# JuliaMolSim/Molly.jl

Measured on AMD Instinct MI355X. Metric: ns_per_day, higher is better.
Workload: dtype f32; 1 GPU; 1M-atom LJ fluid (argon, rho=21.1/nm3), cubic PBC, DistanceCutoff 1.0 nm, r_list 1.2 nm, dt 2 fs, VelocityVerlet, remove_CM_motion=1; integrator=vv, n_atoms=1000000, rebuild_every=10, parallelism=single domain, block_atoms=256, j_split=2, pairs_half_list=75841147

## Files before the change

### molly.jl_amd/csrc/engine.hip

```cpp
#include <algorithm>
#include <chrono>
#include <cstddef>
#include <cstdlib>
#include <cstring>
#include <limits>
#include <memory>
#include <new>
#include <string>
#include <vector>

#include <unistd.h>

#include "bonded.h"
#include "stochastic.h"
#include "constraints.h"
#include "virtual_sites.h"
#include "pme.h"
#include "step_fused.h"
#include "hilbert.h"
#include "kernels.h"
#include "list_policy.h"
#include "replan.h"
#include "halo_step.h"
#include "forces_launch.h"
// ... 715 lines not shown
        case MHIP_COUL_PLAIN: go(std::integral_constant<int, MHIP_COUL_PLAIN>{}); break;
        case MHIP_COUL_REACTION_FIELD: go(std::integral_constant<int, MHIP_COUL_REACTION_FIELD>{}); break;
        default: if (I.approx_erfc) go(std::integral_constant<int, MHIP_COUL_EWALD_DIRECT>{}); else go(std::integral_constant<int, COUL_EWALD_EXACT>{}); break;
        }
    }
    struct PassReq {
        bool step = false;
        bool gcv = false;
        bool cm = false, measure = false;
        double dt = 0;
        const StochP<T>* lang = nullptr;
        bool halo = false, halo_cm_in = false;
        bool fuse_spread = false, fuse_terms = false;
        const double* cm_sum_in = nullptr;
        T4* frc = nullptr;
    };
    struct PassRes {
        bool step = false; int parts = 0;
        bool gs = false, spread = false, terms = false;
        bool cm_summed = false;
    };
    PassShape pass_shape(bool energy, int part, bool allow_gs, const PassReq& req) {
        PassShape s;
        s.fp32 = std::is_same<T, float>::value; s.ljm = ljm; s.coulm = coulm; s.minimg = minimg; s.n_special = n_special > 0 ? 1 : 0; s.eshift = eshift; s.lj_c12 = I.lj_c12 != T(0);
        s.BI = BI; s.JS = JS; s.T_cap = T_cap; s.lds_budget = (size_t)env_int("MOLLYHIP_LDS_BUDGET_KB", 160) * 1024;
        s.dual = dual; s.inner_valid = inner_valid; s.max_tile = max_tile; s.max_tile_in = max_tile_in;
        s.gs = gs_groups(); s.gs_list_current = gs_list_id == n_filters; s.n_ghost = n_ghost;
        s.energy = energy; s.part = part; s.allow_gs = allow_gs; s.own_frc = req.frc != nullptr;
        s.step = req.step; s.halo = req.halo; s.fuse_step = fuse_step_env;
        s.cm_mode = pending_cm.mode(); s.cm_n = pending_cm.n; s.in_step_loop = in_vv_fused || in_lang_fused;
        return s;
    }
    static void throw_capacity(const PassPlan& plan) { if (plan.capacity != PassCapacity::OK) throw ApiError{MHIP_ERR_CAPACITY, capacity_message(plan.capacity)}; }

    PassRes launch_pair_kernel(bool energy, int part = 0, bool allow_gs = false, const PassReq& req = PassReq{}) {
        prune_resolve(!(xf_direct && n_ghost > 0));
        if constexpr (std::is_same<T, float>::value) {
            if (dual && !inner_valid && !energy && allow_gs && part == 0 && !req.frc && adopt_env && gs_groups() > 0 && cnt_outer_valid && margin_zero && !(lp.skin_in < lp.skin)
                && lp.last_outer_step == pass_step && n_ghost == 0 && !host_prune) adopt_outer_list();
        }
        const PassPlan plan = plan_pass(pass_shape(energy, part, allow_gs, req));
        throw_capacity(plan);
        if (req.halo && !plan.steps) throw ApiError{MHIP_ERR_STATE, "internal: the fused ghosted step was asked for a pass that cannot integrate"};
        if (plan.form == PassForm::GROUP_SPLIT) return launch_gs_pass(plan, req);
        last_plan = plan;
        PassRes res;
        ForceArgs<T> A{};
        fill_block_args(A, plan, part, req.frc);
        if (plan.prune) arm_prune(A, plan);
        if (plan.cm_fin) { cm_fin_buf.reserve(4); A.cm_fin_in = pending_cm.parts_arg(); A.cm_fin_n = pending_cm.n; A.cm_fin_out = cm_fin_buf.p; }
        else if (req.cm_sum_in && plan.cm_slot) {
            cm_fin_buf.reserve(4); A.cm_fin_in = req.cm_sum_in; A.cm_fin_n = pending_cm.n; A.cm_fin_out = cm_fin_buf.p; res.cm_summed = true;
        }
        A.dbg = (!plan.prune && !energy) ? stamps_begin((size_t)n_blocks * 16 * 8) : nullptr;
        if (plan.steps) arm_step(A, req);
        prof.begin(plan.prune ? 4 : 0, stream);
        tr(plan.prune ? "k_forces (prune)" : (energy ? "k_forces (energy)" : (plan.steps ? (req.halo ? "k_forces (fused ghosted step)" : "k_forces (fused step)") : "k_forces")));
        launch_block_pass(A, plan, energy, req);
        if (plan.steps) { res.step = true; res.parts = n_blocks; }
        if (plan.cm_fin) pending_cm.moved(cm_fin_buf.p, 1);
        tr("after k_forces");
        if (plan.prune && gs_groups() > 0) {
            regroup(nbr_in.p, cnt_in.p, tile_cnt_in.p, false);
            gs_list_id = n_filters + 1;
        }
        prof.end(plan.prune ? 4 : 0, stream);
        MHIP_HIP(hipGetLastError());
        ++n_force_calls;
        if (A.dbg && (n_force_calls % stamps_every()) == 0) stamps_report();
        if (plan.prune) finish_prune(xf_direct && n_ghost > 0 && prune_late_env);
        return res;
    }

    PassRes launch_gs_pass(const PassPlan& plan, const PassReq& req) {
        PassRes res;
        if constexpr (std::is_same<T, float>::value) {
            const int GS = gs_groups();
            frc_parts.reserve((size_t)(GS - 1) * cap);
            GsArgs Z{};
            Z.G = G; Z.I = I; Z.n_owned = n_owned; Z.BI = BI; Z.BI_shift = ilog2(BI); Z.JS = JS; Z.GS = GS; Z.lgGS = ilog2(GS); Z.R_cap = GS * R_cap;
            Z.T_cap = T_cap; Z.Q_lds = plan.q_lds; Z.n_blocks = n_blocks; Z.spread = std::max(1, n_blocks / GS + 5);
            Z.pos = pos[cur].p; Z.lj = lj[cur].p; Z.tile_idx = inner_is_outer ? tile_idx.p : tile_idx_in.p; Z.tile_cnt = inner_is_outer ? tile_cnt.p : tile_cnt_in.p; Z.nbr = nbr_gs.p; Z.wave_rows = rows_gs.p; Z.blk_center = blk_center.p;
            Z.frc = frc[cur].p; Z.parts = frc_parts.p; Z.part_stride = cap; Z.item_of = gs_item.p;
            Z.dbg = stamps_begin((size_t)n_blocks * GS * 4 * 8);
            last_plan.tile_max = plan.tile_max;
            prof.begin(0, stream);
            tr("k_forces_gs");
            if (req.fuse_spread || req.fuse_terms) {
                bonded.ensure_roles(stream, cap);
                const int order = req.fuse_spread ? pme.order : 5;
                if (plan.cm_fin) cm_fin_buf.reserve(4);
                const size_t lds = (req.fuse_spread ? std::max(plan.lds_bytes, std::min<size_t>((size_t)MAX_LDS_BYTES / GS, spread_head_bytes_f32(order) + (size_t)PME_BOX_BYTES)) : plan.lds_bytes) & ~(size_t)15;
                const int n_spread = req.fuse_spread ? (int)std::min<int64_t>(cdiv(n_owned, (int64_t)64), 4096) : 0;
                launch_pair_spread_bonded(Z, n_blocks * GS, coulm, minimg, order, n_owned, reinterpret_cast<float*>(pme.rgrid.p), reinterpret_cast<const PmeP<float>&>(pme.P), n_spread,
                                          reinterpret_cast<const BondedArgs<float>&>(static_cast<const BondedArgs<T>&>(bonded.slot_args(G, I, pos[cur].p, inv.p))), cdiv(bonded.n_blocks(), 4), lds, stream,
                                          plan.cm_fin ? pending_cm.parts_arg() : (const double*)nullptr, pending_cm.n, plan.cm_fin ? cm_fin_buf.p : (double*)nullptr);
                if (plan.cm_fin) pending_cm.moved(cm_fin_buf.p, 1);
                res.spread = req.fuse_spread; res.terms = !req.fuse_spread;
            } else launch_forces_gs(Z, coulm, minimg, stream);
            prof.end(0, stream);
            MHIP_HIP(hipGetLastError());
            ++n_force_calls; ++n_gs_passes; res.gs = true;
            if (Z.dbg && (n_gs_passes % stamps_every()) == 0) stamps_dump("", (size_t)n_blocks * GS * 4 * 8);
        }
        return res;
    }

    void fill_block_args(ForceArgs<T>& A, const PassPlan& plan, int part, T4* own_frc) {
        A.G = G; A.I = I; A.n_owned = n_owned; A.BI = BI; A.BI_shift = ilog2(BI); A.JS = JS; A.T_cap = T_cap; A.T_lds = plan.tile_lds; A.R_cap = R_cap;
        A.n_blocks = n_blocks; A.blocks_per_xcd = cdiv(n_blocks, 8);
        A.pos = pos[cur].p; A.lj = lj[cur].p; A.blk_center = blk_center.p; A.frc = own_frc ? own_frc : frc[cur].p; A.pe_part = red_part.p;
        const bool pruned = plan.use_inner && !inner_is_outer;
        A.tile_idx = pruned ? tile_idx_in.p : tile_idx.p; A.tile_cnt = pruned ? tile_cnt_in.p : tile_cnt.p;
        A.nbr = pruned ? nbr_in.p : nbr.p; A.wave_rows = pruned ? wave_rows_in.p : wave_rows.p;
        A.r_prune2 = r_prune2; A.any_special = n_special > 0 ? 1 : 0; A.eshift = eshift; A.soa = plan.soa;
        if (part != 0 && !plan.prune) {
            DBuf<int32_t>& fl = plan.use_inner ? blk_ghost_in : blk_ghost; bool& ok = plan.use_inner ? ghost_flags_in_ok : ghost_flags_ok;
            if (!ok) {
                fl.reserve(n_blocks);
                hipLaunchKernelGGL(k_block_ghost_flags, dim3(n_blocks), dim3(WAVE), 0, stream, n_blocks, T_cap, n_owned, (const int32_t*)A.tile_idx, (const int32_t*)A.tile_cnt, fl.p);
                ok = true;
            }
// ... 197 lines not shown
        gs_item.reserve((size_t)n_blocks * GS);
        launch_gs_balance((const int32_t*)rows_gs.p, n_blocks, JS, GS, BI / WAVE, cu_count, gs_item.p, stream);
    }

    void adopt_outer_list() {
        prof.begin(4, stream);
        pos_snap_in.reserve(cap);
        MHIP_HIP(hipMemcpyAsync(pos_snap_in.p, pos[cur].p, (size_t)n_tot * sizeof(T4), hipMemcpyDeviceToDevice, stream));
        regroup(nbr.p, cnt_outer.p, tile_cnt.p, true);
        prof.end(4, stream);
        MHIP_HIP(hipGetLastError());
        inner_is_outer = true; max_tile_in = max_tile; lp.last_prune_step = pass_step;
        ++n_filters; ++n_adopted; gs_list_id = n_filters;
        ghost_flags_in_ok = false; lp.next_check_step = -1; hx.tile_ok = false;
        inner_valid = true; prune_disp_exceeded = false;
        if (debug_on) std::fprintf(stderr, "[mhip] outer list adopted as the inner list (no prune): rows %lld calls %lld\n", (long long)total_rows, (long long)n_force_calls);
    }

#if MHIP_STAMPS
    DBuf<unsigned long long> dbg_buf;
    static int stamps_every() { static const int n = env_int("MOLLYHIP_DBG_TIMES", 0); return std::max(n, 1); }
    unsigned long long* stamps_begin(size_t words) {
        static const int on = env_int("MOLLYHIP_DBG_TIMES", 0);
        if (!on) return nullptr;
        dbg_buf.reserve(words); MHIP_HIP(hipMemsetAsync(dbg_buf.p, 0, words * sizeof(unsigned long long), stream));
        return dbg_buf.p;
    }
    void stamps_dump(const char* suffix, size_t words) {
        std::vector<unsigned long long> h(words);
        MHIP_HIP(hipStreamSynchronize(stream));
        MHIP_HIP(hipMemcpy(h.data(), dbg_buf.p, h.size() * sizeof(unsigned long long), hipMemcpyDeviceToHost));
        if (const char* path = std::getenv("MOLLYHIP_DBG_DUMP")) { if (FILE* f = std::fopen((std::string(path) + suffix).c_str(), "wb")) { std::fwrite(h.data(), sizeof(unsigned long long), h.size(), f); std::fclose(f); } }
    }
    void stamps_report() {
        const int nw = BI * JS / WAVE;
        std::vector<unsigned long long> h((size_t)n_blocks * nw * 8);
        MHIP_HIP(hipStreamSynchronize(stream));
        MHIP_HIP(hipMemcpy(h.data(), dbg_buf.p, h.size() * sizeof(unsigned long long), hipMemcpyDeviceToHost));
        unsigned long long w0 = ~0ull, w3 = 0; double sum[3] = {0, 0, 0}, mx[3] = {0, 0, 0}, clk = 0; int n = 0;
        std::vector<double> loop_us;
        for (size_t q = 0; q < (size_t)n_blocks * nw; ++q) {
            const unsigned long long* d = &h[q * 8];
            if (!d[7]) continue;
            w0 = std::min(w0, d[4]); w3 = std::max(w3, d[7]);
            for (int k = 0; k < 3; ++k) { const double us = (double)(d[5 + k] - d[4 + k]) * 0.01; sum[k] += us; mx[k] = std::max(mx[k], us); }
            loop_us.push_back((double)(d[6] - d[5]) * 0.01);
            if (d[7] > d[4]) clk += (double)(d[3] - d[0]) / ((double)(d[7] - d[4]) * 10.0);
            ++n;
        }
        std::sort(loop_us.begin(), loop_us.end());
        std::fprintf(stderr, "[mhip dbg] pair kernel: %d waves, first entry -> last exit %.2f us | per wave mean (max) us: staging %.2f (%.2f) row walk %.2f (%.2f) reduce+store %.2f (%.2f) | row walk p10 %.2f p50 %.2f p90 %.2f | shader clock %.3f GHz\n",
                     n, (double)(w3 - w0) * 0.01, sum[0] / n, mx[0], sum[1] / n, mx[1], sum[2] / n, mx[2], loop_us[n / 10], loop_us[n / 2], loop_us[(size_t)n * 9 / 10], clk / n);
    }
#else
    static int stamps_every() { return 1; }
    unsigned long long* stamps_begin(size_t) { return nullptr; }
    void stamps_dump(const char*, size_t) {}
    void stamps_report() {}
#endif
    double read_sum(int n_part) {
        hipLaunchKernelGGL(k_sum_double, dim3(1), dim3(256), 0, stream, n_part, (const double*)red_part.p, red_out.p);
        MHIP_HIP(hipMemcpyAsync(h_red, red_out.p, sizeof(double), hipMemcpyDeviceToHost, stream));
        MHIP_HIP(hipStreamSynchronize(stream));
        return h_red[0];
    }

    void export_frc(int accumulate, void* f_xyz, int mem_kind) {
        const size_t cnt = 3 * (size_t)n_owned;
        if (mem_kind == MHIP_MEM_DEVICE) {
            hipLaunchKernelGGL(k_export_forces<T>, dim3(cdiv(n_owned, 256)), dim3(256), 0, stream, n_owned, (const int32_t*)orig[cur].p, (const T4*)frc[cur].p, (T*)f_xyz, accumulate);
        } else {
            stage_a.reserve(cnt);
            if (accumulate) MHIP_HIP(hipMemcpyAsync(stage_a.p, f_xyz, cnt * sizeof(T), hipMemcpyHostToDevice, stream));
            hipLaunchKernelGGL(k_export_forces<T>, dim3(cdiv(n_owned, 256)), dim3(256), 0, stream, n_owned, (const int32_t*)orig[cur].p, (const T4*)frc[cur].p, stage_a.p, accumulate);
            MHIP_HIP(hipMemcpyAsync(f_xyz, stage_a.p, cnt * sizeof(T), hipMemcpyDeviceToHost, stream));
            MHIP_HIP(hipStreamSynchronize(stream));
        }
        MHIP_HIP(hipGetLastError());
    }

    PassRes step_forces(int64_t step_n, PassReq req = PassReq{}) {
        pass_step = step_n;
        if (pme.on() && n_ghost > 0) throw ApiError{MHIP_ERR_UNSUPPORTED, "PME runs on a single domain (SURVEY §8(e): 6mrr-size systems are replicas only)"};
        const bool gs_ok = bonded.any() && n_ghost == 0;
        const bool small_fused = bonded.any() && pme.on() && n_ghost == 0;
        req.fuse_spread = gs_ok && small_fused && pme.order >= 4 && pme.order <= 6 && !prof.on;
        req.fuse_terms = gs_ok && !small_fused && !pme.on() && !prof.on;
        PassRes res = launch_pair_kernel(false, interior_done ? 2 : 0, gs_ok, req);
        interior_done = false;
        bool redo = false;
        if (prune_disp_exceeded) {
            after_forces(step_n);
            req.fuse_spread = req.fuse_terms = false;
            if (res.cm_summed) req.cm_sum_in = nullptr;
            const PassRes again = launch_pair_kernel(false, 0, false, req);
            res.step = again.step; res.parts = again.parts; res.gs = again.gs; res.cm_summed |= again.cm_summed;
            redo = true;
        }
        if (res.gs) bonded.fold(frc_parts.p, gs_groups() - 1, cap);
        pend_a = nullptr;
        if (small_fused) {
            frc_side.reserve(cap);
            GcvArgs<T> V; const GcvArgs<T>* vp = nullptr;
            if (req.gcv && fuse_gcv_env && !redo && (pending_cm.mode() == 0 || (pending_cm.mode() == 2 && pending_cm.n == 1)) && pme.order >= 4 && pme.order <= 6) {
                const int nb = (int)Pme<T>::atom_blocks(n_owned);
                cm_blk.reserve(2 * 4 * (size_t)nb + 8);
                if (req.measure) trk_reserve(nb);
                std::memset(&V, 0, sizeof(V));
                V.vel = vel[cur].p; V.dt = T(req.dt); V.dt2 = T(req.dt) / T(2); V.G = G;
                V.cm_in = pending_cm.parts_arg();
                V.cm_out = req.cm ? cm_blk.p + (size_t)step_half * 4 * nb : (double*)nullptr;
// ... 1681 lines not shown
```

### molly.jl_amd/csrc/kernels.h

```cpp
#pragma once
#include <type_traits>
#include "pass_plan.h"
#include "physics.h"
#include "halo_xfer.h"
#include "philox.h"
#include "thermostat_step.h"

namespace mhip {

enum { FLAG_MINIMG = 0, FLAG_OVERFLOW = 1, FLAG_MAX_TILE = 2, FLAG_MAX_ROWS = 3, FLAG_NAN = 4, FLAG_TOTAL_ROWS = 5, FLAG_MAX_CELLS = 6, FLAG_MAX_DISP2 = 7, FLAG_MAX_V2 = 8, N_FLAGS = 10 };
enum { OVF_TILE = 1, OVF_ROWS = 2, OVF_BOXCELLS = 4, OVF_SLOT = 8 };

constexpr int MAX_BOX_CELLS = 8192;
constexpr uint32_t XL_EXCLUDED = 1u << 30, XL_SPECIAL = 1u << 31, XL_INDEX = (1u << 30) - 1u;

constexpr int SLOT_MAX_SCALED = 16383;
__host__ __device__ inline uint32_t entry_slot(uint32_t e, int sh) { return sh ? (e >> sh) : (e & 0x7fffu); }
__host__ __device__ inline uint32_t entry_special(uint32_t e, int sh) { return sh ? 0u : (e >> 15); }
__host__ __device__ inline uint32_t make_entry(uint32_t slot, uint32_t sp, int sh) { return sh ? (slot << sh) : (slot | (sp << 15)); }

template <class T> __device__ inline int cell_coord(T x, int d, const GridP<T>& G) {
    T rel = G.periodic[d] ? x : x - G.origin[d];
    int c = (int)M<T>::floor(rel * G.inv_cs[d]);
    return min(max(c, 0), G.nc[d] - 1);
// ... 1102 lines not shown
    double a[4] = {0, 0, 0, 0};
    for (int q = threadIdx.x; q < n_part; q += blockDim.x) { const double* p = part + 4 * (int64_t)q; a[0] += p[0]; a[1] += p[1]; a[2] += p[2]; a[3] += p[3]; }
#pragma unroll
    for (int o = 32; o > 0; o >>= 1) for (int c = 0; c < 4; ++c) a[c] += __shfl_xor(a[c], o, 64);
    double* sh = reinterpret_cast<double*>(smem);
    if ((threadIdx.x & 63) == 0) for (int c = 0; c < 4; ++c) sh[4 * (threadIdx.x >> 6) + c] = a[c];
    __syncthreads();
    if (threadIdx.x < 4) { double t = 0; for (int q = 0; q < (int)(blockDim.x >> 6); ++q) t += sh[4 * q + threadIdx.x]; out4[threadIdx.x] = t; }
    __syncthreads();
}

#ifndef MHIP_FAST_MIN_WAVES
#define MHIP_FAST_MIN_WAVES 8
#endif
#ifndef MHIP_SB
#define MHIP_SB 4
#endif
template <class T, int LJM, int COULM, bool ENERGY, bool MINIMG, bool SEG, bool PRUNE>
constexpr int force_min_waves() { return (std::is_same<T, float>::value && LJM == LJ_DIST_UNIFORM && COULM == MHIP_COUL_NONE && !ENERGY && !MINIMG && !SEG && !PRUNE) ? MHIP_FAST_MIN_WAVES : 1; }

template <class T, int LJM, int COULM, bool ENERGY, bool MINIMG, bool SEG, bool PRUNE, int SOA_STRIDE = 4097, bool STEP = false, bool HALO = false, bool LANG = false>
__global__ void __launch_bounds__(BlockLimits<T>::max_threads, (force_min_waves<T, LJM, COULM, ENERGY, MINIMG, SEG, PRUNE>()))
k_forces(ForceArgs<T> A) {
    static_assert(!HALO || (STEP && std::is_same<T, float>::value), "the ghosted form exists for the fused fp32 step only");
    static_assert(!LANG || (STEP && !HALO), "the Langevin update rides in the fused single-domain step only");
    using T4 = typename Vec<T>::T4;
    using T2 = typename Vec<T>::T2;
    constexpr bool PER_ATOM_LJ = (LJM == LJ_DIST || LJM == LJ_GENERIC);
    extern __shared__ __align__(32) unsigned char smem[];
    const GridP<T>& G = A.G;
    int wg = blockIdx.x;
    if constexpr (STEP) {
        if (wg == 0) {
            if constexpr (HALO) { if (A.cm_in) halo_cm_publish(A.H, A.cm_pub, A.step_seq, smem); }
            else if (A.cm_in) step_cm_publish(A.cm_in, A.cm_n, A.cm_pub, A.step_seq, smem);
            return;
        }
        --wg;
    }
    int b = (wg & 7) * A.blocks_per_xcd + (wg >> 3);
    [[maybe_unused]] int hflags = 0;
    if constexpr (HALO) { b = A.H.order[wg]; if (b < 0) return; hflags = A.H.flags[b]; }
    else {
        if (b >= A.n_blocks) return;
        if (A.part != 0 && (A.blk_ghost[b] != 0) != (A.part == 2)) return;
    }
    const int tid = threadIdx.x, nthr = blockDim.x;
    [[maybe_unused]] auto stamp = [&](int k) {
        if constexpr (MHIP_STAMPS != 0 && !PRUNE) {
            if (A.dbg && (tid & 63) == 0) { unsigned long long* d = A.dbg + ((size_t)b * (nthr >> 6) + (tid >> 6)) * 8; d[k] = __builtin_readcyclecounter(); d[4 + k] = wall_clock64(); }
        }
    };
    stamp(0);
    const int tile_n = A.tile_cnt[b];
    T4* l_pos = reinterpret_cast<T4*>(smem);
    T2* l_lj = reinterpret_cast<T2*>(l_pos + (A.T_lds + 1));
    const T4 ctr = A.blk_center[b];
    constexpr bool MAY_SCALE = std::is_same<T, float>::value && LJM == LJ_DIST_UNIFORM && COULM == MHIP_COUL_NONE;
    const int esh = MAY_SCALE ? A.eshift : 0;

    auto localise = [&](T4 p, auto tri_tag) -> T4 {
        if constexpr (!MINIMG) local_xyz_t<decltype(tri_tag)::value>(p.x, p.y, p.z, ctr, G);
        return p;
    };
    constexpr bool NO_TRI = std::is_same<T, float>::value && LJM == LJ_DIST_UNIFORM && COULM == MHIP_COUL_NONE && !ENERGY;
    const bool tri_local = !MINIMG && !NO_TRI && G.tri_grid;
    const int li = tid & (A.BI - 1), js = tid >> A.BI_shift;
    const int64_t si = (int64_t)b * A.BI + li;
    const bool valid = si < A.n_owned;
    [[maybe_unused]] auto step_lane = [&]() -> int { int t = tid; asm volatile("" : "+v"(t)); return t & (A.BI - 1); };
    [[maybe_unused]] auto step_atom = [&]() -> int64_t { return (int64_t)b * A.BI + step_lane(); };
    T4 pi_raw;
    if constexpr (PRUNE || COULM != MHIP_COUL_NONE) pi_raw = A.pos[valid ? si : (int64_t)b * A.BI];
    else {
        const T* own = reinterpret_cast<const T*>(A.pos + (valid ? si : (int64_t)b * A.BI));
        pi_raw = make4<T>(own[0], own[1], own[2], T(0));
    }
    T4 pi;
    T2 lji_raw = make2<T>(T(0), T(0)), lji = lji_raw;
    if constexpr (PER_ATOM_LJ) lji_raw = A.lj[valid ? si : (int64_t)b * A.BI];
    constexpr bool PRE_E = PER_ATOM_LJ && sizeof(T) == 4;
    auto pre_e = [](T2 v) { if constexpr (PRE_E) { v.y = v.x == T(0) ? T(0) : M<T>::sqrt(v.y); v.x *= T(0.5); } return v; };
    const int rows_lane = A.wave_rows[(b * A.JS + js) * (A.BI >> 6) + (li >> 6)];
    int rows = 0;
    bool own_done = false;
    auto own_ready = [&]() {
        if (own_done) return;
        own_done = true;
        if constexpr (NO_TRI) pi = localise(pi_raw, std::false_type{});
        else pi = tri_local ? localise(pi_raw, std::true_type{}) : localise(pi_raw, std::false_type{});
        lji = pre_e(lji_raw);
        rows = __builtin_amdgcn_readfirstlane(rows_lane);
    };
    if constexpr (PRUNE) own_ready();
    const uint2* my_rows = A.nbr + (((int64_t)b * A.JS + js) * A.R_cap) * A.BI + li;
    const int32_t* tix = (HALO ? A.H.tsrc : A.tile_idx) + (int64_t)b * A.T_cap;
    if constexpr (HALO) { if (hflags & 1) halo_wait_block(A.H); }
    T fx = T(0), fy = T(0), fz = T(0), pe = T(0);
    [[maybe_unused]] T vir[6] = {T(0), T(0), T(0), T(0), T(0), T(0)};
    uint64_t acc = 0;
    int kept = 0;
    uint2* out_rows = nullptr;
    if constexpr (PRUNE) out_rows = A.nbr_dst + (((int64_t)b * A.JS + js) * A.R_cap) * A.BI + li;
    [[maybe_unused]] uint16_t* l_new = nullptr; [[maybe_unused]] int32_t* l_scan = nullptr; [[maybe_unused]] float* l_box = nullptr;
    [[maybe_unused]] int32_t* l_cnt = nullptr; [[maybe_unused]] int32_t* l_wmax = nullptr; [[maybe_unused]] const uint2* l_lut = nullptr;
    [[maybe_unused]] int n_new = 0;
// ... 65 lines not shown
                        if constexpr (HALO) {
                            if (s[k] >= 0) p[k] = A.pos[s[k]];
                            else { const float* gr = A.H.rows + 3 * (size_t)(-1 - s[k]); p[k] = make4<T>((T)peer_row_load(gr), (T)peer_row_load(gr + 1), (T)peer_row_load(gr + 2), T(0)); }
                        } else p[k] = A.pos[s[k]];
                    }
#pragma unroll
                    for (int k = 0; k < SB; ++k) {
                        const int t = t0 + k * nthr + tid;
                        if (t < n_here) {
                            const T4 pl = localise(p[k], tri_tag);
                            if (packed3) { l_p3[t] = (float)pl.x; l_p3[SOA_STRIDE + t] = (float)pl.y; l_p3[2 * SOA_STRIDE + t] = (float)pl.z; }
                            else l_pos[t] = pl;
                        }
                    }
                };
                round(0);
                for (int t0 = SB * nthr; t0 < n_here; t0 += SB * nthr) round(t0);
                return;
            }
            for (int t0 = 0; t0 < n_here; t0 += SB * nthr) {
                int s[SB]; T4 p[SB]; [[maybe_unused]] T2 q[SB];
                constexpr bool GUARD = !(FAST_CT && !PRUNE);
                const int kmax = GUARD ? min(SB, (n_here - t0 + nthr - 1) / nthr) : SB;
#pragma unroll
                for (int k = 0; k < SB; ++k) {
                    if (k < kmax) {
                        const int t = min(t0 + k * nthr + tid, n_here - 1);
                        s[k] = tix[seg_lo + t];
                    }
                }
#pragma unroll
                for (int k = 0; k < SB; ++k) if (k < kmax) { p[k] = A.pos[s[k]]; if constexpr (PER_ATOM_LJ) q[k] = A.lj[s[k]]; }
#pragma unroll
                for (int k = 0; k < SB; ++k) {
                    const int t = t0 + k * nthr + tid;
                    if (k < kmax && t < n_here) {
                        const T4 pl = localise(p[k], tri_tag);
                        if (packed3) { l_p3[t] = (float)pl.x; l_p3[SOA_STRIDE + t] = (float)pl.y; l_p3[2 * SOA_STRIDE + t] = (float)pl.z; }
                        else l_pos[t] = pl;
                        if constexpr (PER_ATOM_LJ) l_lj[t] = pre_e(q[k]);
                    }
                }
            }
        };
        if constexpr (NO_TRI) stage(std::false_type{});
        else { if (tri_local) stage(std::true_type{}); else stage(std::false_type{}); }
        own_ready();
        if (tid == 0) {
            if (packed3) { l_p3[n_here] = 1e4f; l_p3[SOA_STRIDE + n_here] = 1e4f; l_p3[2 * SOA_STRIDE + n_here] = 1e4f; }
            else l_pos[n_here] = make4<T>(T(1e4), T(1e4), T(1e4), T(0));
            if constexpr (PER_ATOM_LJ) l_lj[n_here] = make2<T>(T(0), T(0));
        }
        __syncthreads();
        if constexpr (PRUNE) {
            constexpr int NW = 8;
            const float reach2 = (float)A.r_prune2 * 1.001f + 1e-12f;
            const float bL[3] = {(float)G.L[0], (float)G.L[1], (float)G.L[2]}, biL[3] = {(float)G.invL[0], (float)G.invL[1], (float)G.invL[2]};
            auto stays = [&](int t) -> bool {
                if constexpr (MINIMG) { if (G.triclinic) return true; }
                float p[3];
                if (packed3) { p[0] = l_p3[t]; p[1] = l_p3[SOA_STRIDE + t]; p[2] = l_p3[2 * SOA_STRIDE + t]; }
                else { const T4 q = l_pos[t]; p[0] = (float)q.x; p[1] = (float)q.y; p[2] = (float)q.z; }
                float best = 3.0e38f;
#pragma unroll 1
                for (int w = 0; w < NW; ++w) {
                    const float4 lo = reinterpret_cast<const float4*>(l_box)[2 * w], hi = reinterpret_cast<const float4*>(l_box)[2 * w + 1];
                    float ex, ey, ez;
                    if constexpr (MINIMG) {
                        const float blo[3] = {lo.x, lo.y, lo.z}, bhi[3] = {hi.x, hi.y, hi.z};
                        float e[3];
#pragma unroll
                        for (int d = 0; d < 3; ++d) {
                            float dd = p[d] - 0.5f * (blo[d] + bhi[d]);
                            if (G.periodic[d]) dd -= bL[d] * rintf(dd * biL[d]);
                            e[d] = fmaxf(fabsf(dd) - 0.5f * (bhi[d] - blo[d]) - 1e-5f * bL[d], 0.f);
                        }
                        ex = e[0]; ey = e[1]; ez = e[2];
                    } else {
                        ex = fmaxf(fmaxf(lo.x - p[0], p[0] - hi.x), 0.f); ey = fmaxf(fmaxf(lo.y - p[1], p[1] - hi.y), 0.f); ez = fmaxf(fmaxf(lo.z - p[2], p[2] - hi.z), 0.f);
                    }
                    best = fminf(best, ex * ex + ey * ey + ez * ez);
                }
                return best <= reach2;
            };
            const int per = (n_here + nthr - 1) / nthr, t0 = min(tid * per, n_here), t1 = min(t0 + per, n_here);
            int cnt = 0;
            uint32_t keep_bits = 0;
            for (int t = t0; t < t1; ++t) { const bool k = stays(t); cnt += k ? 1 : 0; if (t - t0 < 32) keep_bits |= (k ? 1u : 0u) << (t - t0); }
            l_scan[tid] = cnt;
            __syncthreads();
            if (tid < WAVE) {
                int run = 0;
                for (int base = 0; base < nthr; base += WAVE) {
                    int v = (base + tid < nthr) ? l_scan[base + tid] : 0, x = v;
#pragma unroll
                    for (int o = 1; o < WAVE; o <<= 1) { int u = __shfl_up(x, o, WAVE); if (tid >= o) x += u; }
                    if (base + tid < nthr) l_scan[base + tid] = run + x - v;
                    run += __shfl(x, WAVE - 1, WAVE);
                }
                if (tid == 0) l_scan[nthr] = run;
            }
            __syncthreads();
            {
                int run = n_new + l_scan[tid];
                for (int t = t0; t < t1; ++t) {
                    if ((t - t0 < 32) ? ((keep_bits >> (t - t0)) & 1u) != 0u : stays(t)) { l_new[t] = (uint16_t)(packed3 ? run << ESHIFT_SCALED : run); A.tile_idx_dst[(int64_t)b * A.T_cap + run] = tix[seg_lo + t]; ++run; }
                    else l_new[t] = (uint16_t)0xffffu;
                }
            }
            n_new += l_scan[nthr];
            __syncthreads();
        }
        stamp(1);
        auto walk_rows = [&](auto spec_tag) {
            constexpr bool SPEC = decltype(spec_tag)::value;
            if constexpr (FAST_CT && !SPEC) { if (packed3) {
                typedef float v2f __attribute__((ext_vector_type(2)));
                const v2f pix = {(float)pi.x, (float)pi.x}, piy = {(float)pi.y, (float)pi.y}, piz = {(float)pi.z, (float)pi.z};
                const float c6 = (float)A.I.lj_c6, c12 = (float)A.I.lj_c12, rc2 = (float)A.I.lj_rc2, rp2 = (float)A.r_prune2;
                const float rc2n = __int_as_float(__float_as_int(rc2) + 1);
                const v2f cut_a = {-0x1p100f, -0x1p100f}, cut_b = {rc2n * 0x1p100f, rc2n * 0x1p100f};
                const v2f c48v = {c12, c12}, c24v = {c6, c6};
                v2f fx2 = {(float)fx, 0.f}, fy2 = {(float)fy, 0.f}, fz2 = {(float)fz, 0.f};
                typedef __attribute__((address_space(3))) const char* lds_cptr;
                const lds_cptr lbase = (lds_cptr)(uintptr_t)0;
                auto lds3 = [&](uint32_t oa, uint32_t ob, v2f& dx, v2f& dy, v2f& dz) {
                    typedef __attribute__((address_space(3))) const float* lds_fptr;
                    const lds_fptr pa = (lds_fptr)(lbase + oa), pb = (lds_fptr)(lbase + ob);
                    dx = (v2f){pa[0], pb[0]} - pix; dy = (v2f){pa[SOA_STRIDE], pb[SOA_STRIDE]} - piy; dz = (v2f){pa[2 * SOA_STRIDE], pb[2 * SOA_STRIDE]} - piz;
                };
                auto row = [&](const uint2 e4) {
                    const uint32_t oa = e4.x & 0xffffu, ob = e4.x >> 16, oc = e4.y & 0xffffu, od = e4.y >> 16;
                    v2f dx0, dy0, dz0, dx1, dy1, dz1;
                    lds3(oa, ob, dx0, dy0, dz0); lds3(oc, od, dx1, dy1, dz1);
                    __builtin_amdgcn_sched_group_barrier(0x100, 12, 0);
                    const v2f r20 = __builtin_elementwise_fma(dz0, dz0, __builtin_elementwise_fma(dy0, dy0, dx0 * dx0));
                    const v2f r21 = __builtin_elementwise_fma(dz1, dz1, __builtin_elementwise_fma(dy1, dy1, dx1 * dx1));
                    if constexpr (PRUNE) {
                        typedef __attribute__((address_space(3))) const unsigned short* lds_hptr;
                        auto new_entry = [&](uint32_t o) -> uint32_t { return (uint32_t)*(lds_hptr)(lbase + prune_mark_ct(SOA_STRIDE) + (o >> 1)); };
                        const uint32_t na = new_entry(oa), nb = new_entry(ob), nc = new_entry(oc), nd = new_entry(od);
                        emit4(na, nb, nc, nd, r20.x <= rp2, r20.y <= rp2, r21.x <= rp2, r21.y <= rp2);
                    }
                    const float t0 = __builtin_amdgcn_rcpf(r20.x * r20.y), t1 = __builtin_amdgcn_rcpf(r21.x * r21.y);
                    const v2f u0 = (v2f){r20.y, r20.x} * t0, u1 = (v2f){r21.y, r21.x} * t1;
                    v2f in0, in1;
                    asm("v_pk_fma_f32 %0, %1, %2, %3 clamp\n\ts_nop 0" : "=v"(in0) : "v"(r20), "s"(cut_a), "v"(cut_b));
                    asm("v_pk_fma_f32 %0, %1, %2, %3 clamp\n\ts_nop 0" : "=v"(in1) : "v"(r21), "s"(cut_a), "v"(cut_b));
                    const v2f q0 = u0 * u0, q1 = u1 * u1;
                    const v2f w0 = u0 * in0, w1 = u1 * in1;
                    const v2f c0 = q0 * u0, c1 = q1 * u1;
                    const v2f g0 = __builtin_elementwise_fma(c0, c48v, -c24v), g1 = __builtin_elementwise_fma(c1, c48v, -c24v);
                    const v2f h0 = c0 * w0, h1 = c1 * w1;
                    const v2f f0 = g0 * h0, f1 = g1 * h1;
                    fx2 -= dx0 * f0; fy2 -= dy0 * f0; fz2 -= dz0 * f0;
                    fx2 -= dx1 * f1; fy2 -= dy1 * f1; fz2 -= dz1 * f1;
                };
                if (rows > 0) {
                    const int last = rows - 1;
                    constexpr int D = 2;
                    uint2 e[D] = {my_rows[0], my_rows[(int64_t)min(1, last) * A.BI]};
                    auto next = [&](int q) -> uint2 { return my_rows[(int64_t)min(q, last) * A.BI]; };
                    int r = 0;
                    for (; r + D <= rows; r += D) {
#pragma unroll
                        for (int k = 0; k < D; ++k) { row(e[k]); e[k] = next(r + D + k); }
// ... 33 lines not shown
                        const v2f qa = da * da, qb = db * db;
                        v2f r2 = {__builtin_fmaf(dza, dza, qa.x + qa.y), __builtin_fmaf(dzb, dzb, qb.x + qb.y)};
                        if constexpr (MINIMG) { if (G.triclinic) { if (!real_a) r2.x = 1.0e12f; if (!real_b) r2.y = 1.0e12f; } }
                        if constexpr (PRUNE) {
                            if (valid && real_a && r2.x <= (float)A.r_prune2) emit(make_entry((uint32_t)l_new[sa], 0u, 0));
                            if (valid && real_b && r2.y <= (float)A.r_prune2) emit(make_entry((uint32_t)l_new[sb], 0u, 0));
                        }
                        const v2f fr = pair_eval2<COULM>(reinterpret_cast<const InterP<float>&>(A.I), K, r2, kqi, (v2f){pa.w, pb.w}, si, (v2f){la.x, lb.x}, ei24, (v2f){la.y, lb.y});
                        fxy += da * (v2f){fr.x, fr.x}; fxy += db * (v2f){fr.y, fr.y};
                        fzs = __builtin_fmaf(dza, fr.x, __builtin_fmaf(dzb, fr.y, fzs));
                    }
                    fx -= (T)fxy.x; fy -= (T)fxy.y; fz -= (T)fzs;
                }
            };
            uint2 e_next = (0 < rows) ? my_rows[0] : make_uint2(0, 0);
            constexpr int UNROLL = (sizeof(T) == 8 && (COULM == MHIP_COUL_EWALD_DIRECT || COULM == COUL_EWALD_EXACT)) ? (MINIMG ? 1 : (LJM == LJ_GENERIC && ENERGY ? 2 : 4)) : 4;
            for (int r = 0; r < rows; ++r) {
                const uint2 e4 = e_next;
                if (r + 1 < rows) e_next = my_rows[(int64_t)(r + 1) * A.BI];
                if constexpr (PK2) {
                    if (pk2_ok && (!SPEC || __builtin_amdgcn_ballot_w64(((e4.x | e4.y) & 0x80008000u) != 0u) == 0ull)) { row_pk2(e4); continue; }
                }
#pragma unroll UNROLL
                for (int k = 0; k < 4; ++k) {
                    uint32_t e = ((k < 2 ? e4.x : e4.y) >> (16 * (k & 1))) & 0xffffu;
                    uint32_t slot = entry_slot(e, esh);
                    [[maybe_unused]] const bool real = SEG ? (slot - (uint32_t)seg_lo) < (uint32_t)n_here : slot < (uint32_t)tile_n;
                    if constexpr (SEG) { slot -= (uint32_t)seg_lo; slot = slot < (uint32_t)n_here ? slot : (uint32_t)n_here; }
                    const bool special = SPEC ? entry_special(e, esh) != 0 : false;
                    T4 pj = l_pos[slot];
                    T2 ljj = make2<T>(T(0), T(0));
                    if constexpr (PER_ATOM_LJ) ljj = l_lj[slot];
                    T dx, dy, dz;
                    if constexpr (MINIMG) {
                        min_image_exact<T>(pi.x, pi.y, pi.z, pj.x, pj.y, pj.z, G, dx, dy, dz);
                    } else { dx = pj.x - pi.x; dy = pj.y - pi.y; dz = pj.z - pi.z; }
                    T r2 = dx * dx + dy * dy + dz * dz;
                    if constexpr (MINIMG) { if (G.triclinic && !real) r2 = T(1.0e30); }
                    if constexpr (PRUNE) { if (real && valid && r2 <= A.r_prune2) emit(make_entry((uint32_t)l_new[slot], entry_special(e, esh), esh)); }
                    T fr = pair_eval<T, LJM, COULM, ENERGY, PRE_E>(A.I, r2, pi.w, pj.w, lji.x, ljj.x, lji.y, ljj.y, special, pe);
                    fx -= fr * dx; fy -= fr * dy; fz -= fr * dz;
                    if constexpr (ENERGY) {
                        vir[0] += fr * dx * dx; vir[1] += fr * dy * dy; vir[2] += fr * dz * dz;
                        vir[3] += fr * dx * dy; vir[4] += fr * dx * dz; vir[5] += fr * dy * dz;
                    }
                }
            }
        };
        if constexpr (LJM == LJ_DIST_UNIFORM && COULM == MHIP_COUL_NONE && !ENERGY) {
            if (A.any_special) walk_rows(std::true_type{}); else walk_rows(std::false_type{});
        } else walk_rows(std::true_type{});
        if constexpr (!SEG) break;
    }
    if constexpr (PRUNE) {
        const uint32_t SENTP = make_entry((uint32_t)n_new, 0u, esh);
        const int NWB = A.BI >> 6;
        const bool level = A.level_pairs && A.JS == 2;
        if (level) {
            if (kept & 3) out_rows[(int64_t)(kept >> 2) * A.BI] = make_uint2((uint32_t)acc, (uint32_t)(acc >> 32));
            l_cnt[tid] = kept;
            __syncthreads();
            const int kp = l_cnt[tid ^ A.BI], total = kept + kp, mine = js == 0 ? (total + 1) >> 1 : total >> 1;
            if (kept > mine) {
                uint16_t* to = reinterpret_cast<uint16_t*>(A.nbr_dst + (((int64_t)b * A.JS + (js ^ 1)) * A.R_cap) * A.BI + li);
                const uint16_t* from = reinterpret_cast<const uint16_t*>(out_rows);
                for (int q = 0; q < kept - mine; ++q) {
                    const int ps = mine + q, pd = kp + q;
                    to[(((int64_t)(pd >> 2) * A.BI) << 2) + (pd & 3)] = from[(((int64_t)(ps >> 2) * A.BI) << 2) + (ps & 3)];
                }
            }
            kept = mine;
        }
        if (A.cnt_dst) A.cnt_dst[((int64_t)b * A.JS + js) * A.BI + li] = (uint16_t)min(kept, 65535);
        atomicMax(&l_wmax[js * NWB + (li >> 6)], (kept + 3) >> 2);
        __syncthreads();
        const int rows_wave = l_wmax[js * NWB + (li >> 6)];
        if (level) {
            uint16_t* mine16 = reinterpret_cast<uint16_t*>(out_rows);
            for (int p2 = kept; p2 < 4 * rows_wave; ++p2) mine16[(((int64_t)(p2 >> 2) * A.BI) << 2) + (p2 & 3)] = (uint16_t)SENTP;
        } else
        while (((kept + 3) >> 2) < rows_wave || (kept & 3)) emit(SENTP);
        if (tid < A.JS * NWB) A.rows_dst[b * A.JS * NWB + tid] = l_wmax[tid];
        if (tid == 0) A.tile_cnt_dst[b] = n_new;
        float d2 = 0.f;
        if (valid && js == 0) {
            T4 q = A.pos_snap[si];
            T ex = pi_raw.x - q.x, ey = pi_raw.y - q.y, ez = pi_raw.z - q.z;
            disp_image(ex, ey, ez, G);
            d2 = (float)(ex * ex + ey * ey + ez * ez);
        }
        d2 = wave_max(d2);
        if (js == 0 && (tid & 63) == 0) A.blk_disp2[b * (A.BI >> 6) + (li >> 6)] = d2;
    }
    stamp(2);
    [[maybe_unused]] T4 st_v, st_p;
    [[maybe_unused]] int64_t se = 0;
    [[maybe_unused]] unsigned long long st_w[3] = {0, 0, 0};
    [[maybe_unused]] int snd0 = 0, snd1 = 0;
    if constexpr (STEP) {
        __builtin_amdgcn_s_setprio(3);
        se = step_atom();
        if constexpr (HALO) { if ((hflags & 2) && js == 0 && se < A.n_owned) { snd0 = A.H.snd_start[se]; snd1 = A.H.snd_start[se + 1]; } }
        if (js == 0 && se < A.n_owned) {
            st_v = A.vel[se]; st_p = A.pos[se];
            if (A.cm_in) {
#pragma unroll
                for (int c = 0; c < 3; ++c) st_w[c] = __hip_atomic_load(&A.cm_pub[c], __ATOMIC_RELAXED, __HIP_MEMORY_SCOPE_AGENT);
            }
        }
    }
    if (A.JS > 1) {
        __syncthreads();
        T* red = reinterpret_cast<T*>(smem);
        red[(js * 4 + 0) * A.BI + li] = fx; red[(js * 4 + 1) * A.BI + li] = fy;
        red[(js * 4 + 2) * A.BI + li] = fz; red[(js * 4 + 3) * A.BI + li] = pe;
        __syncthreads();
        if (js == 0) {
            for (int q = 1; q < A.JS; ++q) {
                fx += red[(q * 4 + 0) * A.BI + li]; fy += red[(q * 4 + 1) * A.BI + li];
                fz += red[(q * 4 + 2) * A.BI + li]; pe += red[(q * 4 + 3) * A.BI + li];
            }
        }
    }
    if constexpr (STEP) {
        double px = 0, py = 0, pz = 0, pm = 0;
        float tr_a = 0.f, tr_b = 0.f, tr_v = 0.f;
        T4 v = st_v, p = st_p;
        const bool mine = js == 0 && se < A.n_owned;
        if (mine) {
            if (A.cm_in) {
                if constexpr (HALO) {
                    if ((uint32_t)(st_w[0] >> 32) != A.step_seq || (uint32_t)(st_w[1] >> 32) != A.step_seq || (uint32_t)(st_w[2] >> 32) != A.step_seq) {
// ... 32 lines not shown
            if (A.trk_part) {
                tr_v = (float)(v.x * v.x + v.y * v.y + v.z * v.z);
                auto q = A.snap_a[se];
                T ex = p.x - q.x, ey = p.y - q.y, ez = p.z - q.z;
                disp_image(ex, ey, ez, G);
                tr_a = (float)(ex * ex + ey * ey + ez * ez);
                q = A.snap_b[se];
                ex = p.x - q.x; ey = p.y - q.y; ez = p.z - q.z;
                disp_image(ex, ey, ez, G);
                tr_b = (float)(ex * ex + ey * ey + ez * ez);
            }
        }
        if (A.cm_out || A.trk_part) {
            if (A.JS == 1 && A.BI > 64) __syncthreads();
            double* shd = reinterpret_cast<double*>(smem + (((size_t)A.JS * 4 * A.BI * sizeof(T) + 15) & ~(size_t)15));
            const int le = step_lane(), nw = A.BI >> 6, w = le >> 6, ln = le & 63;
            float* shf = reinterpret_cast<float*>(shd + 16 * nw);
            if (js == 0) {
                if (A.cm_out) { const double sv = row_sum4(px, py, pz, pm, ln); if ((ln & 15) < 4) shd[(w * 4 + (ln >> 4)) * 4 + (ln & 3)] = sv; }
                if (A.trk_part) { const float mv = row_max3(tr_a, tr_b, tr_v, ln); if ((ln & 15) < 3) shf[(w * 4 + (ln >> 4)) * 4 + (ln & 3)] = mv; }
            }
            __syncthreads();
            if (A.cm_out && tid < 4) {
                double a = 0;
                for (int q = 0; q < nw; ++q) { const double* r4 = shd + 16 * q + tid; a += (r4[0] + r4[4]) + (r4[8] + r4[12]); }
                if constexpr (HALO) __hip_atomic_store(&A.cm_out[4 * (int64_t)b + tid], a, __ATOMIC_RELAXED, __HIP_MEMORY_SCOPE_AGENT);
                else A.cm_out[4 * (int64_t)b + tid] = a;
            }
            if (A.trk_part && tid < 3) { float mm = 0.f; for (int q = 0; q < 4 * nw; ++q) mm = fmaxf(mm, shf[4 * q + tid]); A.trk_part[(int64_t)tid * A.n_blocks + b] = mm; }
        }
        if (mine) { A.vel[se] = v; A.pos_next[se] = p; }
        if constexpr (HALO) {
            if (js == 0) {
                if (hflags & 2) {
                    if (!(hflags & 1)) { const int ln = tid & 63; if (ln < A.H.n_peers && !xfer_wait(&A.H.seq_in[A.H.peers[ln]], A.H.seq_wait, A.H.err, A.H.ticks, (9 << 8) | A.H.peers[ln])) atomicOr(A.H.err, 1); }
                    if (mine) for (int r = snd0; r < snd1; ++r) {
                        const HaloSend e = A.H.snd[r];
                        float* d = e.dst + (int64_t)A.H.parity_send * A.H.half_stride;
                        __hip_atomic_store(d, (float)p.x + e.sx, __ATOMIC_RELAXED, __HIP_MEMORY_SCOPE_SYSTEM);
                        __hip_atomic_store(d + 1, (float)p.y + e.sy, __ATOMIC_RELAXED, __HIP_MEMORY_SCOPE_SYSTEM);
                        __hip_atomic_store(d + 2, (float)p.z + e.sz, __ATOMIC_RELAXED, __HIP_MEMORY_SCOPE_SYSTEM);
                    }
                }
                asm volatile("s_waitcnt vmcnt(0)" ::: "memory");
                unsigned int before = 0;
                if ((tid & 63) == 0) before = __hip_atomic_fetch_add(A.H.done, 1u, __ATOMIC_RELAXED, __HIP_MEMORY_SCOPE_AGENT);
                before = (unsigned int)__builtin_amdgcn_readfirstlane((int)before);
                if (before == A.H.n_done - 1u) halo_tail(A.H, A.cm_out, A.n_blocks);
            }
        }
    } else {
        if (js == 0 && valid) A.frc[si] = make4<T>(fx, fy, fz, T(0));
    }
    stamp(3);
    if constexpr (!ENERGY) {
        if (A.cm_fin_out && wg == 0) { __syncthreads(); cm_finalize_in_block(A.cm_fin_in, A.cm_fin_n, A.cm_fin_out, smem); }
    }
    if constexpr (ENERGY) {
        if (A.JS > 1) {
            T* red = reinterpret_cast<T*>(smem);
#pragma unroll
            for (int half = 0; half < 2; ++half) {
                __syncthreads();
#pragma unroll
                for (int c = 0; c < 3; ++c) red[(js * 4 + c) * A.BI + li] = vir[3 * half + c];
                __syncthreads();
                if (js == 0) for (int q = 1; q < A.JS; ++q) for (int c = 0; c < 3; ++c) vir[3 * half + c] += red[(q * 4 + c) * A.BI + li];
            }
        }
        __syncthreads();
        double* dred = reinterpret_cast<double*>(smem);
        for (int c = 0; c < 7; ++c) {
            if (js == 0) dred[li] = valid ? 0.5 * (double)(c == 0 ? pe : vir[c - 1]) : 0.0;
            __syncthreads();
            if (tid == 0) { double s = 0; for (int q = 0; q < A.BI; ++q) s += dred[q]; A.pe_part[(int64_t)c * A.n_blocks + b] = s; }
            __syncthreads();
        }
    }
}

template <class T>
__global__ void k_export_nl(int n_blocks, int BI, int JS, int T_cap, int R_cap, int64_t n_owned, const int32_t* __restrict__ orig,
                            const int32_t* __restrict__ tile_idx, const int32_t* __restrict__ tile_cnt, const uint2* __restrict__ nbr,
                            const int32_t* __restrict__ wave_rows, int32_t* out_i, int32_t* out_j, uint8_t* out_sp,
                            unsigned long long* counter, unsigned long long capacity, int eshift) {
    int b = blockIdx.x, li = threadIdx.x;
    int64_t si = (int64_t)b * BI + li;
    if (si >= n_owned) return;
    int tile_n = tile_cnt[b];
    int oi = orig[si];
    for (int js = 0; js < JS; ++js) {
        int rows = wave_rows[(b * JS + js) * (BI >> 6) + (li >> 6)];
        for (int r = 0; r < rows; ++r) {
            uint2 e4 = nbr[(((int64_t)b * JS + js) * R_cap + r) * BI + li];
            for (int k = 0; k < 4; ++k) {
                uint32_t e = ((k < 2 ? e4.x : e4.y) >> (16 * (k & 1))) & 0xffffu;
                int slot = (int)entry_slot(e, eshift);
                if (slot >= tile_n) continue;
                int oj = orig[tile_idx[(int64_t)b * T_cap + slot]];
                if (oi < oj) {
                    unsigned long long at = atomicAdd(counter, 1ull);
                    if (out_i && at < capacity) { out_i[at] = oi; out_j[at] = oj; out_sp[at] = (uint8_t)entry_special(e, eshift); }
                }
            }
        }
    }
}
// ... 373 lines not shown
```

Measured before the change: 1404 ns/day.

## Restructure prune tile marking with wave ballots and vectorize row padding

The pruning pass's tile-survival marking now assigns tiles round-robin across threads, records keep decisions as wave ballots and scans per-wave popcounts, replacing the contiguous per-thread chunks and per-thread scan. The eight bounding boxes are held in registers and the box loop is unrolled in the non-segmented case. Row relocation is batched four entries at a time, and sentinel padding writes whole uint2 rows instead of individual 16-bit entries. Debug timestamps and a report for the prune pass are also added, compiled only when stamps are enabled. The register-cached boxes raise register pressure in the prune kernel.

After: 1433 ns/day, median of 6. 1.02x the previous value.

```diff
diff --git a/molly.jl_amd/csrc/engine.hip b/molly.jl_amd/csrc/engine.hip
--- a/molly.jl_amd/csrc/engine.hip
+++ b/molly.jl_amd/csrc/engine.hip
@@ -791,7 +791,7 @@
         else if (req.cm_sum_in && plan.cm_slot) {
             cm_fin_buf.reserve(4); A.cm_fin_in = req.cm_sum_in; A.cm_fin_n = pending_cm.n; A.cm_fin_out = cm_fin_buf.p; res.cm_summed = true;
         }
-        A.dbg = (!plan.prune && !energy) ? stamps_begin((size_t)n_blocks * 16 * 8) : nullptr;
+        A.dbg = !energy ? stamps_begin((size_t)n_blocks * 16 * 8) : nullptr;
         if (plan.steps) arm_step(A, req);
         prof.begin(plan.prune ? 4 : 0, stream);
         tr(plan.prune ? "k_forces (prune)" : (energy ? "k_forces (energy)" : (plan.steps ? (req.halo ? "k_forces (fused ghosted step)" : "k_forces (fused step)") : "k_forces")));
@@ -806,7 +806,8 @@
         prof.end(plan.prune ? 4 : 0, stream);
         MHIP_HIP(hipGetLastError());
         ++n_force_calls;
-        if (A.dbg && (n_force_calls % stamps_every()) == 0) stamps_report();
+        if (A.dbg && plan.prune) stamps_report_prune();
+        else if (A.dbg && (n_force_calls % stamps_every()) == 0) stamps_report();
         if (plan.prune) finish_prune(xf_direct && n_ghost > 0 && prune_late_env);
         return res;
     }
@@ -1110,11 +1111,29 @@
         std::fprintf(stderr, "[mhip dbg] pair kernel: %d waves, first entry -> last exit %.2f us | per wave mean (max) us: staging %.2f (%.2f) row walk %.2f (%.2f) reduce+store %.2f (%.2f) | row walk p10 %.2f p50 %.2f p90 %.2f | shader clock %.3f GHz\n",
                      n, (double)(w3 - w0) * 0.01, sum[0] / n, mx[0], sum[1] / n, mx[1], sum[2] / n, mx[2], loop_us[n / 10], loop_us[n / 2], loop_us[(size_t)n * 9 / 10], clk / n);
     }
+    void stamps_report_prune() {
+        const int nw = BI * JS / WAVE;
+        std::vector<unsigned long long> h((size_t)n_blocks * nw * 8);
+        MHIP_HIP(hipStreamSynchronize(stream));
+        MHIP_HIP(hipMemcpy(h.data(), dbg_buf.p, h.size() * sizeof(unsigned long long), hipMemcpyDeviceToHost));
+        unsigned long long w0 = ~0ull, w4 = 0; double sum[4] = {0, 0, 0, 0}, mx[4] = {0, 0, 0, 0}; int n = 0;
+        for (size_t q = 0; q < (size_t)n_blocks * nw; ++q) {
+            const unsigned long long* d = &h[q * 8];
+            if (!d[4]) continue;
+            w0 = std::min(w0, d[0]); w4 = std::max(w4, d[4]);
+            for (int k = 0; k < 4; ++k) { const double us = (double)(d[k + 1] - d[k]) * 0.01; sum[k] += us; mx[k] = std::max(mx[k], us); }
+            ++n;
+        }
+        if (!n) return;
+        std::fprintf(stderr, "[mhip dbg] pruning pass: %d waves, first entry -> last exit %.2f us | per wave mean (max) us: staging %.2f (%.2f) pre-marking %.2f (%.2f) row walk %.2f (%.2f) tail %.2f (%.2f) | sum %.2f\n",
+                     n, (double)(w4 - w0) * 0.01, sum[0] / n, mx[0], sum[1] / n, mx[1], sum[2] / n, mx[2], sum[3] / n, mx[3], (sum[0] + sum[1] + sum[2] + sum[3]) / n);
+    }
 #else
     static int stamps_every() { return 1; }
     unsigned long long* stamps_begin(size_t) { return nullptr; }
     void stamps_dump(const char*, size_t) {}
     void stamps_report() {}
+    void stamps_report_prune() {}
 #endif
     double read_sum(int n_part) {
         hipLaunchKernelGGL(k_sum_double, dim3(1), dim3(256), 0, stream, n_part, (const double*)red_part.p, red_out.p);
diff --git a/molly.jl_amd/csrc/kernels.h b/molly.jl_amd/csrc/kernels.h
--- a/molly.jl_amd/csrc/kernels.h
+++ b/molly.jl_amd/csrc/kernels.h
@@ -1178,6 +1178,12 @@
         }
     };
     stamp(0);
+    [[maybe_unused]] auto pstamp = [&](int k) {
+        if constexpr (MHIP_STAMPS != 0 && PRUNE) {
+            if (A.dbg && (tid & 63) == 0) A.dbg[((size_t)b * (nthr >> 6) + (tid >> 6)) * 8 + k] = wall_clock64();
+        }
+    };
+    pstamp(0);
     const int tile_n = A.tile_cnt[b];
     T4* l_pos = reinterpret_cast<T4*>(smem);
     T2* l_lj = reinterpret_cast<T2*>(l_pos + (A.T_lds + 1));
@@ -1349,22 +1355,38 @@
             if constexpr (PER_ATOM_LJ) l_lj[n_here] = make2<T>(T(0), T(0));
         }
         __syncthreads();
+        pstamp(1);
         if constexpr (PRUNE) {
             constexpr int NW = 8;
             const float reach2 = (float)A.r_prune2 * 1.001f + 1e-12f;
             const float bL[3] = {(float)G.L[0], (float)G.L[1], (float)G.L[2]}, biL[3] = {(float)G.invL[0], (float)G.invL[1], (float)G.invL[2]};
+            [[maybe_unused]] float bx[NW][6];
+#pragma unroll
+            for (int w = 0; w < (SEG ? 0 : NW); ++w) {
+                const float4 lo = reinterpret_cast<const float4*>(l_box)[2 * w], hi = reinterpret_cast<const float4*>(l_box)[2 * w + 1];
+                const float v[6] = {lo.x, lo.y, lo.z, hi.x, hi.y, hi.z};
+#pragma unroll
+                for (int c = 0; c < 6; ++c) bx[w][c] = v[c];
+            }
             auto stays = [&](int t) -> bool {
                 if constexpr (MINIMG) { if (G.triclinic) return true; }
                 float p[3];
                 if (packed3) { p[0] = l_p3[t]; p[1] = l_p3[SOA_STRIDE + t]; p[2] = l_p3[2 * SOA_STRIDE + t]; }
                 else { const T4 q = l_pos[t]; p[0] = (float)q.x; p[1] = (float)q.y; p[2] = (float)q.z; }
                 float best = 3.0e38f;
-#pragma unroll 1
+                constexpr int BOX_UNROLL = SEG ? 1 : NW;
+#pragma unroll BOX_UNROLL
                 for (int w = 0; w < NW; ++w) {
-                    const float4 lo = reinterpret_cast<const float4*>(l_box)[2 * w], hi = reinterpret_cast<const float4*>(l_box)[2 * w + 1];
+                    float blo[3], bhi[3];
+                    if constexpr (SEG) {
+                        const float4 lo = reinterpret_cast<const float4*>(l_box)[2 * w], hi = reinterpret_cast<const float4*>(l_box)[2 * w + 1];
+                        blo[0] = lo.x; blo[1] = lo.y; blo[2] = lo.z; bhi[0] = hi.x; bhi[1] = hi.y; bhi[2] = hi.z;
+                    } else {
+#pragma unroll
+                        for (int d = 0; d < 3; ++d) { blo[d] = bx[w][d]; bhi[d] = bx[w][3 + d]; }
+                    }
                     float ex, ey, ez;
                     if constexpr (MINIMG) {
-                        const float blo[3] = {lo.x, lo.y, lo.z}, bhi[3] = {hi.x, hi.y, hi.z};
                         float e[3];
 #pragma unroll
                         for (int d = 0; d < 3; ++d) {
@@ -1374,41 +1396,52 @@
                         }
                         ex = e[0]; ey = e[1]; ez = e[2];
                     } else {
-                        ex = fmaxf(fmaxf(lo.x - p[0], p[0] - hi.x), 0.f); ey = fmaxf(fmaxf(lo.y - p[1], p[1] - hi.y), 0.f); ez = fmaxf(fmaxf(lo.z - p[2], p[2] - hi.z), 0.f);
+                        ex = fmaxf(fmaxf(blo[0] - p[0], p[0] - bhi[0]), 0.f); ey = fmaxf(fmaxf(blo[1] - p[1], p[1] - bhi[1]), 0.f); ez = fmaxf(fmaxf(blo[2] - p[2], p[2] - bhi[2]), 0.f);
                     }
                     best = fminf(best, ex * ex + ey * ey + ez * ez);
                 }
                 return best <= reach2;
             };
-            const int per = (n_here + nthr - 1) / nthr, t0 = min(tid * per, n_here), t1 = min(t0 + per, n_here);
-            int cnt = 0;
-            uint32_t keep_bits = 0;
-            for (int t = t0; t < t1; ++t) { const bool k = stays(t); cnt += k ? 1 : 0; if (t - t0 < 32) keep_bits |= (k ? 1u : 0u) << (t - t0); }
-            l_scan[tid] = cnt;
-            __syncthreads();
-            if (tid < WAVE) {
-                int run = 0;
-                for (int base = 0; base < nthr; base += WAVE) {
-                    int v = (base + tid < nthr) ? l_scan[base + tid] : 0, x = v;
-#pragma unroll
-                    for (int o = 1; o < WAVE; o <<= 1) { int u = __shfl_up(x, o, WAVE); if (tid >= o) x += u; }
-                    if (base + tid < nthr) l_scan[base + tid] = run + x - v;
-                    run += __shfl(x, WAVE - 1, WAVE);
+            const int nwv = nthr >> 6, wv = tid >> 6;
+            for (int c0 = 0; c0 < n_here; c0 += 64 * nthr) {
+                const int rounds = (min(n_here - c0, 64 * nthr) + nthr - 1) / nthr, cells = rounds * nwv;
+                uint64_t keep_bits = 0;
+                for (int i = 0; i < rounds; ++i) {
+                    const int t = c0 + i * nthr + tid;
+                    const bool k = stays(min(t, n_here)) && t < n_here;
+                    const unsigned long long kept_wave = __builtin_amdgcn_ballot_w64(k);
+                    keep_bits |= (uint64_t)(k ? 1u : 0u) << i;
+                    if ((tid & 63) == 0) l_scan[i * nwv + wv] = __builtin_popcountll(kept_wave);
                 }
-                if (tid == 0) l_scan[nthr] = run;
-            }
-            __syncthreads();
-            {
-                int run = n_new + l_scan[tid];
-                for (int t = t0; t < t1; ++t) {
-                    if ((t - t0 < 32) ? ((keep_bits >> (t - t0)) & 1u) != 0u : stays(t)) { l_new[t] = (uint16_t)(packed3 ? run << ESHIFT_SCALED : run); A.tile_idx_dst[(int64_t)b * A.T_cap + run] = tix[seg_lo + t]; ++run; }
-                    else l_new[t] = (uint16_t)0xffffu;
+                __syncthreads();
+                if (tid < WAVE) {
+                    int run = 0;
+                    for (int base = 0; base < cells; base += WAVE) {
+                        int v = (base + tid < cells) ? l_scan[base + tid] : 0, x = v;
+#pragma unroll
+                        for (int o = 1; o < WAVE; o <<= 1) { int u = __shfl_up(x, o, WAVE); if (tid >= o) x += u; }
+                        if (base + tid < cells) l_scan[base + tid] = run + x - v;
+                        run += __shfl(x, WAVE - 1, WAVE);
+                    }
+                    if (tid == 0) l_scan[nthr] = run;
                 }
-            }
-            n_new += l_scan[nthr];
-            __syncthreads();
-        }
-        stamp(1);
+                __syncthreads();
+                for (int i = 0; i < rounds; ++i) {
+                    const int t = c0 + i * nthr + tid;
+                    const bool k = ((keep_bits >> i) & 1ull) != 0ull;
+                    const unsigned long long kept_wave = __builtin_amdgcn_ballot_w64(k);
+                    if (t < n_here) {
+                        if (k) {
+                            const int run = n_new + l_scan[i * nwv + wv] + (int)__builtin_amdgcn_mbcnt_hi((uint32_t)(kept_wave >> 32), __builtin_amdgcn_mbcnt_lo((uint32_t)kept_wave, 0u));
+                            l_new[t] = (uint16_t)(packed3 ? run << ESHIFT_SCALED : run); A.tile_idx_dst[(int64_t)b * A.T_cap + run] = tix[seg_lo + t];
+                        } else l_new[t] = (uint16_t)0xffffu;
+                    }
+                }
+                n_new += l_scan[nthr];
+                __syncthreads();
+            }
+        }
+        stamp(1); pstamp(2);
         auto walk_rows = [&](auto spec_tag) {
             constexpr bool SPEC = decltype(spec_tag)::value;
             if constexpr (FAST_CT && !SPEC) { if (packed3) {
@@ -1548,6 +1581,7 @@
         } else walk_rows(std::true_type{});
         if constexpr (!SEG) break;
     }
+    pstamp(3);
     if constexpr (PRUNE) {
         const uint32_t SENTP = make_entry((uint32_t)n_new, 0u, esh);
         const int NWB = A.BI >> 6;
@@ -1560,9 +1594,14 @@
             if (kept > mine) {
                 uint16_t* to = reinterpret_cast<uint16_t*>(A.nbr_dst + (((int64_t)b * A.JS + (js ^ 1)) * A.R_cap) * A.BI + li);
                 const uint16_t* from = reinterpret_cast<const uint16_t*>(out_rows);
-                for (int q = 0; q < kept - mine; ++q) {
-                    const int ps = mine + q, pd = kp + q;
-                    to[(((int64_t)(pd >> 2) * A.BI) << 2) + (pd & 3)] = from[(((int64_t)(ps >> 2) * A.BI) << 2) + (ps & 3)];
+                const int rs = A.BI << 2, n_move = kept - mine;
+                auto at = [&](int p) -> int { return (p >> 2) * rs + (p & 3); };
+                for (int q = 0; q < n_move; q += 4) {
+                    uint16_t v[4];
+#pragma unroll
+                    for (int k = 0; k < 4; ++k) v[k] = from[at(mine + min(q + k, n_move - 1))];
+#pragma unroll
+                    for (int k = 0; k < 4; ++k) if (q + k < n_move) to[at(kp + q + k)] = v[k];
                 }
             }
             kept = mine;
@@ -1572,8 +1611,11 @@
         __syncthreads();
         const int rows_wave = l_wmax[js * NWB + (li >> 6)];
         if (level) {
-            uint16_t* mine16 = reinterpret_cast<uint16_t*>(out_rows);
-            for (int p2 = kept; p2 < 4 * rows_wave; ++p2) mine16[(((int64_t)(p2 >> 2) * A.BI) << 2) + (p2 & 3)] = (uint16_t)SENTP;
+            uint16_t* part = reinterpret_cast<uint16_t*>(out_rows + (int64_t)(kept >> 2) * A.BI);
+            for (int c = kept & 3; c != 0 && c < 4; ++c) part[c] = (uint16_t)SENTP;
+            const uint32_t pad2 = (SENTP & 0xffffu) * 0x10001u;
+            uint2* pr = out_rows + (int64_t)((kept + 3) >> 2) * A.BI;
+            for (int q = (kept + 3) >> 2; q < rows_wave; ++q, pr += A.BI) *pr = make_uint2(pad2, pad2);
         } else
         while (((kept + 3) >> 2) < rows_wave || (kept & 3)) emit(SENTP);
         if (tid < A.JS * NWB) A.rows_dst[b * A.JS * NWB + tid] = l_wmax[tid];
@@ -1712,7 +1754,7 @@
     } else {
         if (js == 0 && valid) A.frc[si] = make4<T>(fx, fy, fz, T(0));
     }
-    stamp(3);
+    stamp(3); pstamp(4);
     if constexpr (!ENERGY) {
         if (A.cm_fin_out && wg == 0) { __syncthreads(); cm_finalize_in_block(A.cm_fin_in, A.cm_fin_n, A.cm_fin_out, smem); }
     }
```
